# ntc-ai/sliders-conceptmod

Measured on AMD Instinct MI355X. Metric: slider train-steps/sec (4-pass UNet fwd+bwd), higher is better.
Workload: dtype fp16; 1 GPU; sdxl_1024_b2_r4; unet=sdxl, resolution=1024, per_gpu_batch=2, unet_batch=4, global_batch=2, lora_rank=4, train_method=noxattn, network_type=lierla, lora_params=2662400, scheduler=euler_a, parallelism=dp1, pre_roll=excluded, skip_dead_cfg_half=False, dedup_uncond=False, guidance_passes=1 batched UNet call (3 frozen + 1 adapted sub-batches)

## Files before the change

include/smi.h:

```cpp
#ifndef SMI_H_
#define SMI_H_

#include <stddef.h>
#include <stdint.h>

#ifdef __cplusplus
extern "C" {
#endif

#define SMI_MAX_LEVELS 8
#define SMI_DTYPE_F16 0
#define SMI_DTYPE_BF16 1

typedef struct smi_unet_config {
  int dtype;
  int in_channels;
  int out_channels;
  int n_levels;
  int block_out_channels[SMI_MAX_LEVELS];
  int down_has_attn[SMI_MAX_LEVELS];
  int up_has_attn[SMI_MAX_LEVELS];
  int layers_per_block;
  int transformer_layers[SMI_MAX_LEVELS];
  int num_heads[SMI_MAX_LEVELS];
// ... 259 lines not shown
int smi_op_conv3x3(int dtype, const void* in, const void* w_packed, const void* bias, void* out, int nb, int hin,
                   int win, int cin, int cout, int stride, int upsample, int transposed, int hout, int wout,
                   void* stream);
int smi_op_upconv_phase(int dtype, const void* in, const void* w, const void* bias, void* wph, void* planes, void* out, int nb,
                        int h, int w_, int cin, int cout, int tile_code, int* ran_code, void* stream);
int smi_set_upconv_phase(int on);
int smi_op_attention_fwd(int dtype, const void* q, const void* k, const void* v, void* o, float* lse, int b, int h,
                         int nq, int nk, int d, float scale, void* stream);
int smi_op_attention_bwd(int dtype, const void* q, const void* k, const void* v, const void* o, const float* lse,
                         const void* d_o, void* dq, void* dk, void* dv, float* delta, int b, int h, int nq, int nk,
                         int d, float scale, void* stream);
typedef struct smi_attn_args {
  const void *q, *k, *v;
  void* o;
  float* lse;
  const void* d_o;
  void *dq, *dk, *dv;
  float* delta;
  void* stream;
  int64_t ldq, ldk, ldv, ldo, lddo, lddq, lddk, lddv;
  int dtype, b, h, nq, nk, d;
  float scale;
  int causal, sel_xs, sel_fused;
} smi_attn_args;
#define SMI_ATTN_FWD 1
#define SMI_ATTN_XS_FWD 2
#define SMI_ATTN_BWD_FUSED 3
#define SMI_ATTN_DQ 4
#define SMI_ATTN_XS_DQ 5
#define SMI_ATTN_DKV 6
#define SMI_ATTN_DK_DV 7
#define SMI_ATTN_DELTA 8
typedef struct smi_attn_ran {
  int dp;
  int form;
  int n_launches;
  int family[4];
  int chain;
} smi_attn_ran;
int smi_op_attention_ex_fwd(const smi_attn_args* args, smi_attn_ran* ran);
int smi_op_attention_ex_bwd(const smi_attn_args* args, smi_attn_ran* ran);
int smi_op_attention_causal_fwd(int dtype, const void* q, const void* k, const void* v, void* o, float* lse, int b, int h,
                                int n, int d, int64_t ldq, int64_t ldk, int64_t ldv, int64_t ldo, float scale, void* stream);
int smi_op_attention_causal_bwd(int dtype, const void* q, const void* k, const void* v, const void* o, const float* lse,
                                const void* d_o, void* dq, void* dk, void* dv, float* delta, int b, int h, int nq, int nk,
                                int d, int64_t ldq, int64_t ldk, int64_t ldv, int64_t ldo, int64_t lddo, int64_t lddq,
                                int64_t lddk, int64_t lddv, float scale, void* stream);
int smi_op_act(int dtype, const void* x, void* y, const void* dy, void* dx, int64_t n, int kind, void* stream);
int smi_op_groupnorm(int dtype, const void* x, const void* gamma, const void* beta, void* y, const void* dy, void* dx,
                     float* scratch, int nb, int hw, int c, int g, float eps, int silu, void* stream);
int smi_op_layernorm(int dtype, const void* x, const void* gamma, const void* beta, void* y, const void* dy, void* dx,
                     float* mean_rstd, int m, int c, float eps, void* stream);
typedef struct smi_norm_args {
  const void *x, *gamma, *beta;
  void* y;
  const void *dy, *add;
  void* dx;
  float* scratch;
  void* stream;
  int dtype, nb, hw, c, g;
  float eps;
// ... 98 lines not shown
```

sliders_conceptmod_amd/_native.py:

```python
from __future__ import annotations

import ctypes as C
import os
from typing import List, Optional, Sequence

import torch

_HERE = os.path.dirname(os.path.abspath(__file__))
LIB_PATH = os.environ.get("SMI_LIB") or os.path.join(_HERE, "libsmi_hip.so")
SMI_MAX_LEVELS = 8
DTYPE_CODE = {torch.float16: 0, torch.bfloat16: 1}


class SmiError(RuntimeError):
    pass


class UNetConfigC(C.Structure):
    _fields_ = [
        ("dtype", C.c_int), ("in_channels", C.c_int), ("out_channels", C.c_int), ("n_levels", C.c_int),
        ("block_out_channels", C.c_int * SMI_MAX_LEVELS), ("down_has_attn", C.c_int * SMI_MAX_LEVELS),
        ("up_has_attn", C.c_int * SMI_MAX_LEVELS), ("layers_per_block", C.c_int),
        ("transformer_layers", C.c_int * SMI_MAX_LEVELS), ("num_heads", C.c_int * SMI_MAX_LEVELS),
        ("mid_transformer_layers", C.c_int), ("cross_attention_dim", C.c_int), ("norm_num_groups", C.c_int),
# ... 35 lines not shown
    _fields_ = [("name", C.c_char_p), ("data", C.c_void_p), ("ndim", C.c_int), ("shape", C.c_int64 * 4)]


class LoraSiteC(C.Structure):
    _fields_ = [("target", C.c_char_p), ("off_down", C.c_int64), ("off_up", C.c_int64), ("rank", C.c_int),
                ("scale", C.c_float), ("off_dora", C.c_int64)]


class WgradJobC(C.Structure):
    _fields_ = [("X", C.c_void_p), ("P", C.c_void_p), ("dW", C.c_void_p), ("row_scale", C.c_void_p),
                ("ldx", C.c_int64), ("ldp", C.c_int64), ("so_r", C.c_int64), ("so_k", C.c_int64),
                ("M", C.c_int), ("K", C.c_int), ("r", C.c_int), ("seg_cols", C.c_int), ("rows_per_sample", C.c_int),
                ("alpha", C.c_float), ("m_begin", C.c_int), ("conv_tap", C.c_int), ("Hin", C.c_int), ("Win", C.c_int),
                ("Hout", C.c_int), ("Wout", C.c_int), ("conv_stride", C.c_int), ("conv_ups", C.c_int)]


class AttnArgsC(C.Structure):
    _fields_ = [("q", C.c_void_p), ("k", C.c_void_p), ("v", C.c_void_p), ("o", C.c_void_p), ("lse", C.c_void_p),
                ("d_o", C.c_void_p), ("dq", C.c_void_p), ("dk", C.c_void_p), ("dv", C.c_void_p), ("delta", C.c_void_p),
                ("stream", C.c_void_p),
                ("ldq", C.c_int64), ("ldk", C.c_int64), ("ldv", C.c_int64), ("ldo", C.c_int64), ("lddo", C.c_int64),
                ("lddq", C.c_int64), ("lddk", C.c_int64), ("lddv", C.c_int64),
                ("dtype", C.c_int), ("b", C.c_int), ("h", C.c_int), ("nq", C.c_int), ("nk", C.c_int), ("d", C.c_int),
                ("scale", C.c_float), ("causal", C.c_int), ("sel_xs", C.c_int), ("sel_fused", C.c_int)]


class AttnRanC(C.Structure):
    _fields_ = [("dp", C.c_int), ("form", C.c_int), ("n_launches", C.c_int), ("family", C.c_int * 4), ("chain", C.c_int)]


class NormArgsC(C.Structure):
    _fields_ = [("x", C.c_void_p), ("gamma", C.c_void_p), ("beta", C.c_void_p), ("y", C.c_void_p), ("dy", C.c_void_p),
                ("add", C.c_void_p), ("dx", C.c_void_p), ("scratch", C.c_void_p), ("stream", C.c_void_p),
                ("dtype", C.c_int), ("nb", C.c_int), ("hw", C.c_int), ("c", C.c_int), ("g", C.c_int), ("eps", C.c_float),
                ("silu", C.c_int), ("bwd_n0", C.c_int), ("sel_fused", C.c_int)]


class NormRanC(C.Structure):
    _fields_ = [("form", C.c_int), ("chunks", C.c_int), ("slots", C.c_int), ("nv", C.c_int), ("r", C.c_int)]


class DoraSiteC(C.Structure):
    _fields_ = [("W", C.c_void_p), ("off_down", C.c_int64), ("off_up", C.c_int64), ("off_dora", C.c_int64),
                ("dW", C.c_void_p), ("dWt", C.c_void_p), ("cnorm", C.c_void_p), ("r", C.c_int), ("nseg", C.c_int),
                ("K", C.c_int), ("cs", C.c_int), ("scale", C.c_float)]


class LoraPrepSiteC(C.Structure):
    _fields_ = [("off_down", C.c_int64), ("off_up", C.c_int64), ("dst_down", C.c_int64), ("dst_up", C.c_int64),
                ("r", C.c_int), ("nseg", C.c_int), ("K", C.c_int), ("cs", C.c_int), ("rows_pad", C.c_int), ("conv", C.c_int),
                ("dst_gw", C.c_int64)]
# ... 816 lines not shown
```

sliders_conceptmod_amd/build.py:

```python
import os
import subprocess
import sys

HERE = os.path.dirname(os.path.abspath(__file__))
CSRC = os.path.join(HERE, "csrc")
LIB = os.path.join(HERE, "libsmi_hip.so")
SOURCES = ["gemm.hip", "gemm2.hip", "gemm3.hip", "gemm4.hip", "attention.hip", "attention_causal.hip", "norm.hip", "elementwise.hip", "lora.hip", "vae_decode.hip", "clip_vision.hip",
           "lpips.hip", "mmdit.hip", "engine.hip", "engine_unet.hip", "engine_vae.hip", "engine_clip.hip", "engine_lpips.hip", "engine_mmdit.hip", "ops_api.hip"]
FLAGS = ["--offload-arch=gfx950", "-O3", "-std=c++17", "-fPIC"]
EXTRA_FLAGS = {"attention.hip": ["-mllvm", "-amdgpu-mfma-vgpr-form"],
               "attention_causal.hip": ["-mllvm", "-amdgpu-mfma-vgpr-form"]}


def _stale(target, deps):
    if not os.path.exists(target):
        return True
    t = os.path.getmtime(target)
    return any(os.path.getmtime(d) > t for d in deps)


def build(force: bool = False, verbose: bool = False) -> str:
    hipcc = os.environ.get("HIPCC", "hipcc")
    objdir = os.path.join(HERE, "build")
    os.makedirs(objdir, exist_ok=True)
    headers = [os.path.join(CSRC, h) for h in ("smi_common.h", "kernels.h", "gemm_tile.h", "gemm_epilogue.h", "engine.h")] + [
        os.path.join(os.path.dirname(HERE), "include", "smi.h")]
    objs = []
    procs = []
    for src in SOURCES:
        s = os.path.join(CSRC, src)
        o = os.path.join(objdir, src.replace(".hip", ".o"))
        objs.append(o)
        if force or _stale(o, [s] + headers):
            cmd = [hipcc] + FLAGS + EXTRA_FLAGS.get(src, []) + ["-c", s, "-o", o]
            if verbose:
                print(" ".join(cmd))
            procs.append((src, subprocess.Popen(cmd, stdout=subprocess.PIPE, stderr=subprocess.STDOUT)))
    for src, p in procs:
        out, _ = p.communicate()
        if p.returncode != 0:
            raise RuntimeError(f"hipcc failed on {src}:\n{out.decode()}")
    if force or procs or _stale(LIB, objs):
        cmd = [hipcc, "--offload-arch=gfx950", "-shared", "-fPIC", "-o", LIB] + objs
        r = subprocess.run(cmd, stdout=subprocess.PIPE, stderr=subprocess.STDOUT)
        if r.returncode != 0:
            raise RuntimeError(f"link failed:\n{r.stdout.decode()}")
    return LIB

# ... 4 lines not shown
```

sliders_conceptmod_amd/csrc/attention.hip:

```cpp
#include <stdlib.h>

#include <type_traits>

#include "kernels.h"

namespace smi {
namespace {

constexpr float LOG2E = 1.4426950408889634f;
constexpr int TK = 64;
typedef short s16x4 __attribute__((ext_vector_type(4)));
__host__ __device__ constexpr int tr_stride(int DP) { return ((DP * 2) % 128 == 64) ? DP : DP + 32; }

__device__ __forceinline__ void xcd_block(int& bx, int& by, int& bz) {
  const int nx = gridDim.x, ny = gridDim.y;
  const int total = nx * ny * gridDim.z;
  const int lin = blockIdx.x + nx * (blockIdx.y + ny * blockIdx.z);
  const int q = total >> 3, r = total & 7, xcd = lin & 7;
  const int v = (xcd < r ? xcd * (q + 1) : r * (q + 1) + (xcd - r) * q) + (lin >> 3);
  bx = v % nx;
  const int t = v / nx;
  by = t % ny;
  bz = t / ny;
}

template <typename T, int DP>
struct Stage {
  static constexpr int LDN = DP + 8;
  static constexpr int LDV = tr_stride(DP);
  static constexpr int NIT = DP / 32;
  static constexpr int CPR = DP / 8;

  static __device__ __forceinline__ void load(u32x4 (&reg)[NIT], __amdgpu_buffer_rsrc_t r, int64_t row0, int nrows,
                                              int64_t ld, int col0, int D, int tid) {
#pragma unroll
    for (int i = 0; i < NIT; ++i) {
      const int idx = tid + 256 * i;
      const int row = idx / CPR, ch = idx - row * CPR;
      const bool ok = (row0 + row < nrows) && (ch * 8 < D);
      const uint32_t off = ok ? (uint32_t)(((row0 + row) * ld + col0 + ch * 8) * 2) : OOB;
      reg[i] = buf_load16(r, off);
    }
  }
  static __device__ __forceinline__ void store_nat(const u32x4 (&reg)[NIT], T* dst, int tid) {
#pragma unroll
    for (int i = 0; i < NIT; ++i) {
      const int idx = tid + 256 * i;
      const int row = idx / CPR, ch = idx - row * CPR;
      *reinterpret_cast<u32x4*>(dst + row * LDN + ch * 8) = reg[i];
    }
  }
  static __device__ __forceinline__ void store_ld(const u32x4 (&reg)[NIT], T* dst, int ld, int tid) {
#pragma unroll
    for (int i = 0; i < NIT; ++i) {
      const int idx = tid + 256 * i;
      const int row = idx / CPR, ch = idx - row * CPR;
      *reinterpret_cast<u32x4*>(dst + row * ld + ch * 8) = reg[i];
    }
  }
};

template <typename T>
__device__ __forceinline__ typename TT<T>::v8 pack8(const f32x16& a, int s) {
  Pack8<T> t;
#pragma unroll
  for (int j = 0; j < 8; ++j) t.e[j] = from_f<T>(a[8 * s + j]);
  return t.v;
}
template <typename T>
__device__ __forceinline__ typename TT<T>::v8 ld_frag_nat(const T* tile, int ldn, int row, int col) {
  Pack8<T> t;
  t.u = *reinterpret_cast<const u32x4*>(tile + row * ldn + col);
  return t.v;
}
template <typename T>
__device__ __forceinline__ typename TT<T>::v8 ld_frag_trhw(const T* tile, int ld, int idx0, int d0, int lane) {
  const T* a = tile + (idx0 + ((lane & 15) >> 2)) * ld + d0 + ((lane >> 4) & 1) * 16 + 4 * (lane & 3);
  typedef __attribute__((address_space(3))) s16x4 lds_s16x4;
  const s16x4 lo = __builtin_amdgcn_ds_read_tr16_b64_v4i16((lds_s16x4*)a);
  const s16x4 hi = __builtin_amdgcn_ds_read_tr16_b64_v4i16((lds_s16x4*)(a + 8 * ld));
  union {
    s16x4 h[2];
    typename TT<T>::v8 v;
  } u;
  u.h[0] = lo;
  u.h[1] = hi;
  return u.v;
}

template <typename T> struct Sum4;
template <> struct Sum4<f16> {
  static __device__ __forceinline__ f32x4 add8(f16x8 pf, f32x4 acc) {
    const f16x4 one = {(f16)1.f, (f16)1.f, (f16)1.f, (f16)1.f};
    const f16x4 lo = {pf[0], pf[1], pf[2], pf[3]}, hi = {pf[4], pf[5], pf[6], pf[7]};
    acc = __builtin_amdgcn_mfma_f32_4x4x4f16(one, lo, acc, 0, 0, 0);
    return __builtin_amdgcn_mfma_f32_4x4x4f16(one, hi, acc, 0, 0, 0);
  }
};
template <> struct Sum4<bf16> {
  typedef short s4 __attribute__((ext_vector_type(4)));
  static __device__ __forceinline__ f32x4 add8(bf16x8 pf, f32x4 acc) {
    const s4 one = {0x3F80, 0x3F80, 0x3F80, 0x3F80};
    union { bf16x8 v; s4 h[2]; } u;
    u.v = pf;
    acc = __builtin_amdgcn_mfma_f32_4x4x4bf16_1k(one, u.h[0], acc, 0, 0, 0);
    return __builtin_amdgcn_mfma_f32_4x4x4bf16_1k(one, u.h[1], acc, 0, 0, 0);
  }
};
__device__ __forceinline__ void halves_split(float x, float& lo, float& hi) {
  lo = x;
  hi = x;
  asm volatile("s_nop 1\n\tv_permlane32_swap_b32 %0, %1\n\ts_nop 0" : "+v"(lo), "+v"(hi));
}
__device__ __forceinline__ float halves_max(float x) {
  float a, b;
  halves_split(x, a, b);
  return fmaxf(a, b);
}
__device__ __forceinline__ float halves_sum(float x) {
  float a, b;
  halves_split(x, a, b);
  return a + b;
}
__device__ __forceinline__ int acc_row(int r, int h2) { return (r & 3) + 8 * (r >> 2) + 4 * h2; }

template <typename T, int DP, int NSD>
__global__ __launch_bounds__(256) void attn_fwd_kernel(AttnParams p) {
  using S = Stage<T, DP>;
  constexpr int NS = DP / 16, NB = DP / 32;
  constexpr bool EX = NSD > 0;
  __shared__ __attribute__((aligned(16))) T Ks2[2][TK * S::LDN];
  __shared__ __attribute__((aligned(16))) T Vs2[2][TK * S::LDV];

  const int tid = threadIdx.x, lane = tid & 63, wave = tid >> 6;
  const int ql = lane & 31, h2 = lane >> 5;
  int bx, head, b;
  xcd_block(bx, head, b);
  const int q_idx = bx * 128 + wave * 32 + ql;
  const int col0 = head * p.D;
  const int nsd = NSD > 0 ? NSD : (p.D + 15) / 16;

  const auto rQ = make_rsrc((const T*)p.Q + (int64_t)b * p.Nq * p.ldq, (uint32_t)((int64_t)p.Nq * p.ldq * 2));
  const auto rK = make_rsrc((const T*)p.K + (int64_t)b * p.Nk * p.ldk, (uint32_t)((int64_t)p.Nk * p.ldk * 2));
  const auto rV = make_rsrc((const T*)p.V + (int64_t)b * p.Nk * p.ldv, (uint32_t)((int64_t)p.Nk * p.ldv * 2));

  typename TT<T>::v8 qf[NS];
#pragma unroll
// ... 454 lines not shown
#pragma unroll
      for (int g = 0; g < 4; ++g) {
        const int d = i * 32 + 8 * g + 4 * h2;
        if (d < p.D) {
          if (DO_DK) {
            Pack4<T> t;
#pragma unroll
            for (int j = 0; j < 4; ++j) t.e[j] = from_f<T>(dk[i][4 * g + j] * p.scale);
            *reinterpret_cast<u32x2*>((T*)p.dK + ((int64_t)b * p.Nk + k_idx) * p.lddk + col0 + d) = t.u;
          }
          if (DO_DV) {
            Pack4<T> t;
#pragma unroll
            for (int j = 0; j < 4; ++j) t.e[j] = from_f<T>(dv[i][4 * g + j]);
            *reinterpret_cast<u32x2*>((T*)p.dV + ((int64_t)b * p.Nk + k_idx) * p.lddv + col0 + d) = t.u;
          }
        }
      }
  }
}

constexpr int XS_KEYS = 96;

__device__ __forceinline__ void wave_lds_sync() {
  __builtin_amdgcn_fence(__ATOMIC_ACQ_REL, "wavefront");
  __builtin_amdgcn_wave_barrier();
}

template <typename T, int DP>
struct XsTile {
  static constexpr int LDN = DP + 8;
  static constexpr int CPR = DP / 8;
  static constexpr int TOT = 32 * CPR;
  static constexpr int NIT = TOT / 64;
  static_assert(TOT % 64 == 0, "tile depth");
  static __device__ __forceinline__ void rc(int lane, int i, int& row, int& col) {
    const int idx = lane + 64 * i;
    row = idx / CPR;
    col = (idx - row * CPR) * 8;
  }
  static __device__ __forceinline__ void load(u32x4 (&reg)[NIT], __amdgpu_buffer_rsrc_t r, int64_t row0, int nrows,
                                              int64_t ld, int col0, int D, int lane) {
#pragma unroll
    for (int i = 0; i < NIT; ++i) {
      int row, col;
      rc(lane, i, row, col);
      const bool ok = (row0 + row < nrows) && (col < D);
      reg[i] = buf_load16(r, ok ? (uint32_t)(((row0 + row) * ld + col0 + col) * 2) : OOB);
    }
  }
  static __device__ __forceinline__ void to_lds(const u32x4 (&reg)[NIT], T* tile, int lane) {
// ... 346 lines not shown
  constexpr size_t sm = xs_fwd_smem<T, DP>();
  if (sm > 65536) {
    static DynLdsOnce once;
    if (int rc = once.set((const void*)attn_xs_fwd_kernel<T, DP, NSD>, (int)sm)) return rc;
  }
  dim3 grid(xs_grid_x(p), p.H, p.B);
  hipLaunchKernelGGL((attn_xs_fwd_kernel<T, DP, NSD>), grid, dim3(256), sm, st, p);
  SMI_HIP(hipGetLastError());
  return 0;
}
template <typename T, int DP, int NSD>
int xs_dq_launch(const AttnParams& p, hipStream_t st) {
  constexpr size_t sm = xs_dq_smem<T, DP>();
  if (sm > 65536) {
    static DynLdsOnce once;
    if (int rc = once.set((const void*)attn_xs_bwd_dq_kernel<T, DP, NSD>, (int)sm)) return rc;
  }
  dim3 grid(xs_grid_x(p), p.H, p.B);
  hipLaunchKernelGGL((attn_xs_bwd_dq_kernel<T, DP, NSD>), grid, dim3(256), sm, st, p);
  SMI_HIP(hipGetLastError());
  return 0;
}
static int g_sel_xs = -1, g_sel_fused = -1;
static thread_local AttnRan g_ran;
static void ran_begin(int dp, int form) {
  g_ran = AttnRan();
  g_ran.dp = dp;
  g_ran.form = form;
}
static void ran_add(int family, int chain = 0) {
  if (g_ran.n < 4) g_ran.family[g_ran.n] = family;
  ++g_ran.n;
  if (chain) g_ran.chain = chain;
}
static int xs_chain(const AttnParams& p) { return cdiv(p.Nq, 128) / xs_grid_x(p); }

static bool xs_enabled() {
  static const bool on = []() { const char* e = getenv("SMI_ATTN_XS"); return !(e && e[0] == '0'); }();
  return g_sel_xs < 0 ? on : g_sel_xs != 0;
}

template <typename T, int DP>
constexpr size_t dkv_smem() {
  return (size_t)(2 * TK * Stage<T, DP>::LDN + 2 * TK * Stage<T, DP>::LDV) * sizeof(T) + 2 * TK * sizeof(float);
}
template <typename T, int DP, int WHICH, int NSD>
// ... 11 lines not shown
  const int total = gridDim.x, lin = blockIdx.x;
  const int q = total >> 3, r = total & 7, xcd = lin & 7;
  const int v = (xcd < r ? xcd * (q + 1) : r * (q + 1) + (xcd - r) * q) + (lin >> 3);
  const int bh = v / per, j = v - bh * per;
  const int head = bh % p.H, b = bh / p.H;
  if (j < nkb)
    attn_bwd_dkv_body<T, DP, 3, NSD, true>(p, j, head, b, dyn_smem);
  else
    attn_bwd_dq_body<T, DP, NSD, false>(p, j - nkb, head, b, dyn_smem);
}

int check_attn(const AttnParams& p) {
  SMI_CHECK(p.D % 8 == 0 && p.D >= 8 && p.D <= 160, "attention: head_dim %d unsupported (need D %% 8 == 0, <= 160)", p.D);
  SMI_CHECK(p.ldq % 8 == 0 && p.ldk % 8 == 0 && p.ldv % 8 == 0 && p.ldo % 8 == 0,
            "attention: row strides ldq %lld ldk %lld ldv %lld ldo %lld must be multiples of 8 elements (16 bytes)",
            (long long)p.ldq, (long long)p.ldk, (long long)p.ldv, (long long)p.ldo);
  SMI_CHECK(p.B > 0 && p.H > 0 && p.Nq > 0 && p.Nk > 0, "attention: empty shape");
  SMI_CHECK((int64_t)p.Nq * p.ldq * 2 < 0xFFFFFFF0ll && (int64_t)p.Nk * p.ldk * 2 < 0xFFFFFFF0ll, "attention: per-batch tensor larger than 4 GiB");
  return 0;
}

template <int DP> constexpr int alt_steps() { return DP == 64 ? 3 : (DP == 96 ? 5 : 0); }

template <typename T, int DP>
int fwd_t(const AttnParams& p, hipStream_t st) {
  dim3 grid(cdiv(p.Nq, 128), p.H, p.B);
  constexpr int NS = DP / 16, ALT = alt_steps<DP>();
  const int nsd = (p.D + 15) / 16;
  ran_begin(DP, nsd == NS ? 1 : (ALT > 0 && nsd == ALT ? 2 : 0));
  if (p.Nk <= XS_KEYS && xs_enabled() && g_ran.form != 0) {
    ran_add(ATTN_RAN_XS_FWD, xs_chain(p));
    if (nsd == NS) return xs_fwd_launch<T, DP, NS>(p, st);
    return xs_fwd_launch<T, DP, (ALT > 0 ? ALT : NS)>(p, st);
  }
  ran_add(ATTN_RAN_FWD);
  if (nsd == NS)
    hipLaunchKernelGGL((attn_fwd_kernel<T, DP, NS>), grid, dim3(256), 0, st, p);
  else if (ALT > 0 && nsd == ALT)
    hipLaunchKernelGGL((attn_fwd_kernel<T, DP, (ALT > 0 ? ALT : NS)>), grid, dim3(256), 0, st, p);
  else
    hipLaunchKernelGGL((attn_fwd_kernel<T, DP, 0>), grid, dim3(256), 0, st, p);
  SMI_HIP(hipGetLastError());
  return 0;
}

template <typename T, int DP, int WHICH, int NSD>
int dkv_launch(const AttnParams& p, dim3 grid, size_t sm, hipStream_t st) {
  if (sm > 65536) {
    static DynLdsOnce once;
    if (int rc = once.set((const void*)attn_bwd_dkv_kernel<T, DP, WHICH, NSD>, (int)sm)) return rc;
  }
  hipLaunchKernelGGL((attn_bwd_dkv_kernel<T, DP, WHICH, NSD>), grid, dim3(256), sm, st, p);
  return 0;
}

template <typename T, int DP>
int bwd_t(const AttnParams& p, hipStream_t st) {
  constexpr int NS = DP / 16, ALT = alt_steps<DP>();
// ... 57 lines not shown
      else { if (dkv_launch<T, DP, 3, 0>(p, grid, sm, st)) return -2; }
    } else {
      if (form == 1) {
        if (dkv_launch<T, DP, 1, NS>(p, grid, sm, st) || dkv_launch<T, DP, 2, NS>(p, grid, sm, st)) return -2;
      } else {
        if (dkv_launch<T, DP, 1, 0>(p, grid, sm, st) || dkv_launch<T, DP, 2, 0>(p, grid, sm, st)) return -2;
      }
    }
  }
  SMI_HIP(hipGetLastError());
  return 0;
}

template <typename T>
int dispatch(const AttnParams& p, hipStream_t st, bool bwd) {
  if (p.D <= 32) return bwd ? bwd_t<T, 32>(p, st) : fwd_t<T, 32>(p, st);
  if (p.D <= 64) return bwd ? bwd_t<T, 64>(p, st) : fwd_t<T, 64>(p, st);
  if (p.D <= 96) return bwd ? bwd_t<T, 96>(p, st) : fwd_t<T, 96>(p, st);
  return bwd ? bwd_t<T, 160>(p, st) : fwd_t<T, 160>(p, st);
}

}

void set_attn_select(int xs, int fused) {
  g_sel_xs = xs;
  g_sel_fused = fused;
}
AttnRan attn_last_ran() { return g_ran; }

int launch_attn_fwd(const AttnParams& p, hipStream_t stream) {
  g_ran = AttnRan();
  if (check_attn(p)) return -1;
  return p.dtype == DT_F16 ? dispatch<f16>(p, stream, false) : dispatch<bf16>(p, stream, false);
}
int launch_attn_bwd(const AttnParams& p, hipStream_t stream) {
  g_ran = AttnRan();
  if (p.causal) return launch_attn_causal_bwd(p, stream);
  if (check_attn(p)) return -1;
  SMI_CHECK(p.lse && p.delta && p.dO && p.O, "attention bwd: lse/delta/dO/O required");
  SMI_CHECK(p.lddo % 8 == 0 && (!p.dQ || p.lddq % 8 == 0) && (!p.dK || p.lddk % 8 == 0) && (!p.dV || p.lddv % 8 == 0),
            "attention bwd: row strides lddo %lld lddq %lld lddk %lld lddv %lld must be multiples of 8 elements (16 bytes)",
            (long long)p.lddo, (long long)p.lddq, (long long)p.lddk, (long long)p.lddv);
  return p.dtype == DT_F16 ? dispatch<f16>(p, stream, true) : dispatch<bf16>(p, stream, true);
}

}
```

sliders_conceptmod_amd/csrc/kernels.h:

```cpp
#pragma once
#include <vector>

#include "smi_common.h"

namespace smi {

struct GemmParams {
  int dtype = DT_F16;
  const void* A = nullptr;
  int64_t lda = 0;
  const void* W = nullptr;
  void* C = nullptr;
  int64_t ldc = 0;
  int out_f32 = 0;
  int M = 0, N = 0, K = 0;
  const void* bias = nullptr;
  const void* res = nullptr;
  int64_t ldr = 0;
  const void* rowvec = nullptr;
  int rows_per_vec = 1;
  int64_t ld_rowvec = 0;
  const float* lora_xa = nullptr;
  int64_t ld_xa = 0;
  const float* lora_up = nullptr;
// ... 133 lines not shown
void set_gemm_scratch(void* ws, size_t bytes);
bool gemm_geglu_supported(const GemmParams& p);

int launch_conv3x3_small(int dtype, const void* in, const void* w, const void* bias, void* out, int out_f32, int Nb,
                         int H, int W, int Cin, int Cout, hipStream_t stream);

struct AttnParams {
  int dtype = DT_F16;
  const void *Q = nullptr, *K = nullptr, *V = nullptr;
  void* O = nullptr;
  float* lse = nullptr;
  int64_t ldq = 0, ldk = 0, ldv = 0, ldo = 0;
  int B = 0, H = 0, Nq = 0, Nk = 0, D = 0;
  float scale = 1.f;
  int causal = 0;
  const void* dO = nullptr;
  int64_t lddo = 0;
  float* delta = nullptr;
  void *dQ = nullptr, *dK = nullptr, *dV = nullptr;
  int64_t lddq = 0, lddk = 0, lddv = 0;
};
int launch_attn_fwd(const AttnParams& p, hipStream_t stream);
int launch_attn_bwd(const AttnParams& p, hipStream_t stream);
void set_attn_select(int xs, int fused);
enum {
  ATTN_RAN_FWD = 1,
  ATTN_RAN_XS_FWD = 2,
  ATTN_RAN_BWD_FUSED = 3,
  ATTN_RAN_DQ = 4,
  ATTN_RAN_XS_DQ = 5,
  ATTN_RAN_DKV = 6,
  ATTN_RAN_DK_DV = 7,
  ATTN_RAN_DELTA = 8,
};
struct AttnRan {
  int dp = 0;
  int form = 0;
  int n = 0;
  int family[4] = {0, 0, 0, 0};
  int chain = 0;
};
AttnRan attn_last_ran();
int launch_attn_causal_bwd(const AttnParams& p, hipStream_t stream);

int gn_num_chunks(int HW);
size_t gn_partial_floats(int Nb, int HW, int G);
int launch_groupnorm_fwd(int dtype, const void* x, const void* gamma, const void* beta, void* y, float* ab,
                         float* mean_rstd, float* partial, int Nb, int HW, int C, int G, float eps, int silu,
                         hipStream_t stream);
int launch_groupnorm_stats(int dtype, const void* x, const void* gamma, const void* beta, float* ab, float* mean_rstd,
                           float* partial, int Nb, int HW, int C, int G, float eps, hipStream_t stream);
int launch_groupnorm_bwd(int dtype, const void* x, const void* dy, const void* gamma, const void* beta,
                         const float* a, const float* b, const float* mean_rstd, const void* add, void* dx,
                         float* partial, int Nb, int HW, int C, int G, int silu, hipStream_t stream);
void set_gn_select(int fused);
enum {
  NORM_RAN_GN_ONE = 1,
  NORM_RAN_GN_TWO = 2,
  NORM_RAN_GN_FOLD = 3,
  NORM_RAN_LN = 4,
};
struct NormRan {
  int form = 0;
// ... 192 lines not shown
```

sliders_conceptmod_amd/csrc/ops_api.hip:

```cpp
#include <cstdarg>
#include <cstdio>
#include <cstring>
#include <vector>

#include "../../include/smi.h"
#include "kernels.h"

namespace smi {

static thread_local char g_err[2048] = "";
void set_error(const char* fmt, ...) {
  va_list ap;
  va_start(ap, fmt);
  vsnprintf(g_err, sizeof(g_err), fmt, ap);
  va_end(ap);
}

}

using namespace smi;

extern "C" {

const char* smi_last_error(void) { return g_err; }
// ... 151 lines not shown
  p.B = a->b;
  p.H = a->h;
  p.Nq = a->nq;
  p.Nk = a->nk;
  p.D = a->d;
  p.scale = a->scale;
  p.causal = a->causal;
  p.dO = a->d_o;
  p.lddo = a->lddo;
  p.delta = a->delta;
  p.dQ = a->dq;
  p.dK = a->dk;
  p.dV = a->dv;
  p.lddq = a->lddq;
  p.lddk = a->lddk;
  p.lddv = a->lddv;
  return p;
}
static int attn_ex_run(const smi_attn_args* a, smi_attn_ran* ran, bool bwd) {
  if (!a) {
    set_error("smi_op_attention_ex: NULL arguments");
    return -1;
  }
  set_attn_select(a->sel_xs, a->sel_fused);
  const AttnParams p = attn_ex(a);
  const int rc = bwd ? launch_attn_bwd(p, (hipStream_t)a->stream) : launch_attn_fwd(p, (hipStream_t)a->stream);
  set_attn_select(-1, -1);
  if (ran) {
    const AttnRan r = attn_last_ran();
    ran->dp = r.dp;
    ran->form = r.form;
    ran->n_launches = r.n;
    for (int i = 0; i < 4; ++i) ran->family[i] = r.family[i];
    ran->chain = r.chain;
  }
  return rc;
}
int smi_op_attention_ex_fwd(const smi_attn_args* a, smi_attn_ran* ran) { return attn_ex_run(a, ran, false); }
int smi_op_attention_ex_bwd(const smi_attn_args* a, smi_attn_ran* ran) { return attn_ex_run(a, ran, true); }
static AttnParams attn_causal(int dtype, const void* q, const void* k, const void* v, void* o, float* lse, int b, int h, int n,
                              int d, int64_t ldq, int64_t ldk, int64_t ldv, int64_t ldo, float scale) {
  AttnParams p = attn_dense(dtype, q, k, v, o, lse, b, h, n, n, d, scale);
  p.ldq = ldq;
  p.ldk = ldk;
  p.ldv = ldv;
  p.ldo = ldo;
  p.causal = 1;
  return p;
}
int smi_op_attention_causal_fwd(int dtype, const void* q, const void* k, const void* v, void* o, float* lse, int b, int h,
                                int n, int d, int64_t ldq, int64_t ldk, int64_t ldv, int64_t ldo, float scale, void* stream) {
  return launch_attn_fwd(attn_causal(dtype, q, k, v, o, lse, b, h, n, d, ldq, ldk, ldv, ldo, scale), (hipStream_t)stream);
}
int smi_op_attention_causal_bwd(int dtype, const void* q, const void* k, const void* v, const void* o, const float* lse,
                                const void* d_o, void* dq, void* dk, void* dv, float* delta, int b, int h, int nq, int nk,
                                int d, int64_t ldq, int64_t ldk, int64_t ldv, int64_t ldo, int64_t lddo, int64_t lddq,
                                int64_t lddk, int64_t lddv, float scale, void* stream) {
// ... 391 lines not shown
```

Before: 6.756 steps/s.

## Add 8-wave ping-pong attention forward kernel for head_dim 64 fp16

Adds a 512-thread attention forward kernel where two 4-wave groups alternate, one staging the next K/V tiles into double-buffered LDS while the other runs the QK/PV MFMAs. Each block covers 256 queries instead of 128. A rule picks this kernel for fp16, head_dim 64, at least 256 keys and enough workgroups, with an env switch to turn it off. Shared attention helpers move into a common header. The aim is better overlap of global loads with matrix math, at the cost of more register and LDS pressure and added barrier handshakes.

```diff
diff --git a/include/smi.h b/include/smi.h
--- a/include/smi.h
+++ b/include/smi.h
@@ -305,6 +305,7 @@
   int dtype, b, h, nq, nk, d;
   float scale;
   int causal, sel_xs, sel_fused;
+  int sel_fwd;
 } smi_attn_args;
 #define SMI_ATTN_FWD 1
 #define SMI_ATTN_XS_FWD 2
@@ -320,6 +321,7 @@
   int n_launches;
   int family[4];
   int chain;
+  int fwd;
 } smi_attn_ran;
 int smi_op_attention_ex_fwd(const smi_attn_args* args, smi_attn_ran* ran);
 int smi_op_attention_ex_bwd(const smi_attn_args* args, smi_attn_ran* ran);
diff --git a/sliders_conceptmod_amd/_native.py b/sliders_conceptmod_amd/_native.py
--- a/sliders_conceptmod_amd/_native.py
+++ b/sliders_conceptmod_amd/_native.py
@@ -81,11 +81,13 @@
                 ("ldq", C.c_int64), ("ldk", C.c_int64), ("ldv", C.c_int64), ("ldo", C.c_int64), ("lddo", C.c_int64),
                 ("lddq", C.c_int64), ("lddk", C.c_int64), ("lddv", C.c_int64),
                 ("dtype", C.c_int), ("b", C.c_int), ("h", C.c_int), ("nq", C.c_int), ("nk", C.c_int), ("d", C.c_int),
-                ("scale", C.c_float), ("causal", C.c_int), ("sel_xs", C.c_int), ("sel_fused", C.c_int)]
+                ("scale", C.c_float), ("causal", C.c_int), ("sel_xs", C.c_int), ("sel_fused", C.c_int),
+                ("sel_fwd", C.c_int)]
 
 
 class AttnRanC(C.Structure):
-    _fields_ = [("dp", C.c_int), ("form", C.c_int), ("n_launches", C.c_int), ("family", C.c_int * 4), ("chain", C.c_int)]
+    _fields_ = [("dp", C.c_int), ("form", C.c_int), ("n_launches", C.c_int), ("family", C.c_int * 4), ("chain", C.c_int),
+                ("fwd", C.c_int)]
 
 
 class NormArgsC(C.Structure):
diff --git a/sliders_conceptmod_amd/build.py b/sliders_conceptmod_amd/build.py
--- a/sliders_conceptmod_amd/build.py
+++ b/sliders_conceptmod_amd/build.py
@@ -5,10 +5,11 @@
 HERE = os.path.dirname(os.path.abspath(__file__))
 CSRC = os.path.join(HERE, "csrc")
 LIB = os.path.join(HERE, "libsmi_hip.so")
-SOURCES = ["gemm.hip", "gemm2.hip", "gemm3.hip", "gemm4.hip", "attention.hip", "attention_causal.hip", "norm.hip", "elementwise.hip", "lora.hip", "vae_decode.hip", "clip_vision.hip",
+SOURCES = ["gemm.hip", "gemm2.hip", "gemm3.hip", "gemm4.hip", "attention.hip", "attention_fwd8.hip", "attention_causal.hip", "norm.hip", "elementwise.hip", "lora.hip", "vae_decode.hip", "clip_vision.hip",
            "lpips.hip", "mmdit.hip", "engine.hip", "engine_unet.hip", "engine_vae.hip", "engine_clip.hip", "engine_lpips.hip", "engine_mmdit.hip", "ops_api.hip"]
 FLAGS = ["--offload-arch=gfx950", "-O3", "-std=c++17", "-fPIC"]
 EXTRA_FLAGS = {"attention.hip": ["-mllvm", "-amdgpu-mfma-vgpr-form"],
+               "attention_fwd8.hip": ["-mllvm", "-amdgpu-mfma-vgpr-form"],
                "attention_causal.hip": ["-mllvm", "-amdgpu-mfma-vgpr-form"]}
 
 
@@ -23,7 +24,7 @@
     hipcc = os.environ.get("HIPCC", "hipcc")
     objdir = os.path.join(HERE, "build")
     os.makedirs(objdir, exist_ok=True)
-    headers = [os.path.join(CSRC, h) for h in ("smi_common.h", "kernels.h", "gemm_tile.h", "gemm_epilogue.h", "engine.h")] + [
+    headers = [os.path.join(CSRC, h) for h in ("smi_common.h", "kernels.h", "attention_common.h", "gemm_tile.h", "gemm_epilogue.h", "engine.h")] + [
         os.path.join(os.path.dirname(HERE), "include", "smi.h")]
     objs = []
     procs = []
diff --git a/sliders_conceptmod_amd/csrc/attention.hip b/sliders_conceptmod_amd/csrc/attention.hip
--- a/sliders_conceptmod_amd/csrc/attention.hip
+++ b/sliders_conceptmod_amd/csrc/attention.hip
@@ -2,127 +2,10 @@
 
 #include <type_traits>
 
-#include "kernels.h"
+#include "attention_common.h"
 
 namespace smi {
 namespace {
-
-constexpr float LOG2E = 1.4426950408889634f;
-constexpr int TK = 64;
-typedef short s16x4 __attribute__((ext_vector_type(4)));
-__host__ __device__ constexpr int tr_stride(int DP) { return ((DP * 2) % 128 == 64) ? DP : DP + 32; }
-
-__device__ __forceinline__ void xcd_block(int& bx, int& by, int& bz) {
-  const int nx = gridDim.x, ny = gridDim.y;
-  const int total = nx * ny * gridDim.z;
-  const int lin = blockIdx.x + nx * (blockIdx.y + ny * blockIdx.z);
-  const int q = total >> 3, r = total & 7, xcd = lin & 7;
-  const int v = (xcd < r ? xcd * (q + 1) : r * (q + 1) + (xcd - r) * q) + (lin >> 3);
-  bx = v % nx;
-  const int t = v / nx;
-  by = t % ny;
-  bz = t / ny;
-}
-
-template <typename T, int DP>
-struct Stage {
-  static constexpr int LDN = DP + 8;
-  static constexpr int LDV = tr_stride(DP);
-  static constexpr int NIT = DP / 32;
-  static constexpr int CPR = DP / 8;
-
-  static __device__ __forceinline__ void load(u32x4 (&reg)[NIT], __amdgpu_buffer_rsrc_t r, int64_t row0, int nrows,
-                                              int64_t ld, int col0, int D, int tid) {
-#pragma unroll
-    for (int i = 0; i < NIT; ++i) {
-      const int idx = tid + 256 * i;
-      const int row = idx / CPR, ch = idx - row * CPR;
-      const bool ok = (row0 + row < nrows) && (ch * 8 < D);
-      const uint32_t off = ok ? (uint32_t)(((row0 + row) * ld + col0 + ch * 8) * 2) : OOB;
-      reg[i] = buf_load16(r, off);
-    }
-  }
-  static __device__ __forceinline__ void store_nat(const u32x4 (&reg)[NIT], T* dst, int tid) {
-#pragma unroll
-    for (int i = 0; i < NIT; ++i) {
-      const int idx = tid + 256 * i;
-      const int row = idx / CPR, ch = idx - row * CPR;
-      *reinterpret_cast<u32x4*>(dst + row * LDN + ch * 8) = reg[i];
-    }
-  }
-  static __device__ __forceinline__ void store_ld(const u32x4 (&reg)[NIT], T* dst, int ld, int tid) {
-#pragma unroll
-    for (int i = 0; i < NIT; ++i) {
-      const int idx = tid + 256 * i;
-      const int row = idx / CPR, ch = idx - row * CPR;
-      *reinterpret_cast<u32x4*>(dst + row * ld + ch * 8) = reg[i];
-    }
-  }
-};
-
-template <typename T>
-__device__ __forceinline__ typename TT<T>::v8 pack8(const f32x16& a, int s) {
-  Pack8<T> t;
-#pragma unroll
-  for (int j = 0; j < 8; ++j) t.e[j] = from_f<T>(a[8 * s + j]);
-  return t.v;
-}
-template <typename T>
-__device__ __forceinline__ typename TT<T>::v8 ld_frag_nat(const T* tile, int ldn, int row, int col) {
-  Pack8<T> t;
-  t.u = *reinterpret_cast<const u32x4*>(tile + row * ldn + col);
-  return t.v;
-}
-template <typename T>
-__device__ __forceinline__ typename TT<T>::v8 ld_frag_trhw(const T* tile, int ld, int idx0, int d0, int lane) {
-  const T* a = tile + (idx0 + ((lane & 15) >> 2)) * ld + d0 + ((lane >> 4) & 1) * 16 + 4 * (lane & 3);
-  typedef __attribute__((address_space(3))) s16x4 lds_s16x4;
-  const s16x4 lo = __builtin_amdgcn_ds_read_tr16_b64_v4i16((lds_s16x4*)a);
-  const s16x4 hi = __builtin_amdgcn_ds_read_tr16_b64_v4i16((lds_s16x4*)(a + 8 * ld));
-  union {
-    s16x4 h[2];
-    typename TT<T>::v8 v;
-  } u;
-  u.h[0] = lo;
-  u.h[1] = hi;
-  return u.v;
-}
-
-template <typename T> struct Sum4;
-template <> struct Sum4<f16> {
-  static __device__ __forceinline__ f32x4 add8(f16x8 pf, f32x4 acc) {
-    const f16x4 one = {(f16)1.f, (f16)1.f, (f16)1.f, (f16)1.f};
-    const f16x4 lo = {pf[0], pf[1], pf[2], pf[3]}, hi = {pf[4], pf[5], pf[6], pf[7]};
-    acc = __builtin_amdgcn_mfma_f32_4x4x4f16(one, lo, acc, 0, 0, 0);
-    return __builtin_amdgcn_mfma_f32_4x4x4f16(one, hi, acc, 0, 0, 0);
-  }
-};
-template <> struct Sum4<bf16> {
-  typedef short s4 __attribute__((ext_vector_type(4)));
-  static __device__ __forceinline__ f32x4 add8(bf16x8 pf, f32x4 acc) {
-    const s4 one = {0x3F80, 0x3F80, 0x3F80, 0x3F80};
-    union { bf16x8 v; s4 h[2]; } u;
-    u.v = pf;
-    acc = __builtin_amdgcn_mfma_f32_4x4x4bf16_1k(one, u.h[0], acc, 0, 0, 0);
-    return __builtin_amdgcn_mfma_f32_4x4x4bf16_1k(one, u.h[1], acc, 0, 0, 0);
-  }
-};
-__device__ __forceinline__ void halves_split(float x, float& lo, float& hi) {
-  lo = x;
-  hi = x;
-  asm volatile("s_nop 1\n\tv_permlane32_swap_b32 %0, %1\n\ts_nop 0" : "+v"(lo), "+v"(hi));
-}
-__device__ __forceinline__ float halves_max(float x) {
-  float a, b;
-  halves_split(x, a, b);
-  return fmaxf(a, b);
-}
-__device__ __forceinline__ float halves_sum(float x) {
-  float a, b;
-  halves_split(x, a, b);
-  return a + b;
-}
-__device__ __forceinline__ int acc_row(int r, int h2) { return (r & 3) + 8 * (r >> 2) + 4 * h2; }
 
 template <typename T, int DP, int NSD>
 __global__ __launch_bounds__(256) void attn_fwd_kernel(AttnParams p) {
@@ -623,11 +506,6 @@
 
 constexpr int XS_KEYS = 96;
 
-__device__ __forceinline__ void wave_lds_sync() {
-  __builtin_amdgcn_fence(__ATOMIC_ACQ_REL, "wavefront");
-  __builtin_amdgcn_wave_barrier();
-}
-
 template <typename T, int DP>
 struct XsTile {
   static constexpr int LDN = DP + 8;
@@ -1020,6 +898,7 @@
   return 0;
 }
 static int g_sel_xs = -1, g_sel_fused = -1;
+static int g_sel_fwd = 0;
 static thread_local AttnRan g_ran;
 static void ran_begin(int dp, int form) {
   g_ran = AttnRan();
@@ -1077,6 +956,14 @@
 
 template <int DP> constexpr int alt_steps() { return DP == 64 ? 3 : (DP == 96 ? 5 : 0); }
 
+constexpr int FWD8_MIN_KEYS = 256;
+constexpr int FWD8_MIN_WGS = 1024;
+static bool fwd8_rule(const AttnParams& p) {
+  static const bool on = []() { const char* e = getenv("SMI_ATTN_FWD8"); return !(e && e[0] == '0'); }();
+  if (!on || !attn_fwd8_can(p) || p.dtype != DT_F16) return false;
+  return p.Nk >= FWD8_MIN_KEYS && (int64_t)cdiv(p.Nq, 256) * p.H * p.B >= FWD8_MIN_WGS;
+}
+
 template <typename T, int DP>
 int fwd_t(const AttnParams& p, hipStream_t st) {
   dim3 grid(cdiv(p.Nq, 128), p.H, p.B);
@@ -1084,11 +971,21 @@
   const int nsd = (p.D + 15) / 16;
   ran_begin(DP, nsd == NS ? 1 : (ALT > 0 && nsd == ALT ? 2 : 0));
   if (p.Nk <= XS_KEYS && xs_enabled() && g_ran.form != 0) {
+    SMI_CHECK(g_sel_fwd != 2, "attention: the 8-wave forward was pinned, but %d keys go to the single-pass kernel", p.Nk);
     ran_add(ATTN_RAN_XS_FWD, xs_chain(p));
     if (nsd == NS) return xs_fwd_launch<T, DP, NS>(p, st);
     return xs_fwd_launch<T, DP, (ALT > 0 ? ALT : NS)>(p, st);
   }
   ran_add(ATTN_RAN_FWD);
+  if constexpr (DP == 64) {
+    if (g_sel_fwd == 2 || (g_sel_fwd == 0 && fwd8_rule(p))) {
+      g_ran.fwd = 2;
+      const int rc = launch_attn_fwd8(p, st);
+      if (rc) g_ran = AttnRan();
+      return rc;
+    }
+  }
+  g_ran.fwd = 1;
   if (nsd == NS)
     hipLaunchKernelGGL((attn_fwd_kernel<T, DP, NS>), grid, dim3(256), 0, st, p);
   else if (ALT > 0 && nsd == ALT)
@@ -1192,9 +1089,10 @@
 
 }
 
-void set_attn_select(int xs, int fused) {
+void set_attn_select(int xs, int fused, int fwd) {
   g_sel_xs = xs;
   g_sel_fused = fused;
+  g_sel_fwd = fwd;
 }
 AttnRan attn_last_ran() { return g_ran; }
 
diff --git a/sliders_conceptmod_amd/csrc/attention_common.h b/sliders_conceptmod_amd/csrc/attention_common.h
--- /dev/null
+++ b/sliders_conceptmod_amd/csrc/attention_common.h
@@ -0,0 +1,132 @@
+#pragma once
+
+#include "kernels.h"
+
+namespace smi {
+namespace {
+
+constexpr float LOG2E = 1.4426950408889634f;
+constexpr int TK = 64;
+typedef short s16x4 __attribute__((ext_vector_type(4)));
+__host__ __device__ constexpr int tr_stride(int DP) { return ((DP * 2) % 128 == 64) ? DP : DP + 32; }
+
+__device__ __forceinline__ void xcd_block(int& bx, int& by, int& bz) {
+  const int nx = gridDim.x, ny = gridDim.y;
+  const int total = nx * ny * gridDim.z;
+  const int lin = blockIdx.x + nx * (blockIdx.y + ny * blockIdx.z);
+  const int q = total >> 3, r = total & 7, xcd = lin & 7;
+  const int v = (xcd < r ? xcd * (q + 1) : r * (q + 1) + (xcd - r) * q) + (lin >> 3);
+  bx = v % nx;
+  const int t = v / nx;
+  by = t % ny;
+  bz = t / ny;
+}
+
+template <typename T, int DP, int NT = 256>
+struct Stage {
+  static constexpr int LDN = DP + 8;
+  static constexpr int LDV = tr_stride(DP);
+  static constexpr int NIT = TK * DP / 8 / NT;
+  static constexpr int CPR = DP / 8;
+  static_assert(NIT * NT * 8 == TK * DP, "tile chunks must divide among the threads");
+
+  static __device__ __forceinline__ void load(u32x4 (&reg)[NIT], __amdgpu_buffer_rsrc_t r, int64_t row0, int nrows,
+                                              int64_t ld, int col0, int D, int tid) {
+#pragma unroll
+    for (int i = 0; i < NIT; ++i) {
+      const int idx = tid + NT * i;
+      const int row = idx / CPR, ch = idx - row * CPR;
+      const bool ok = (row0 + row < nrows) && (ch * 8 < D);
+      const uint32_t off = ok ? (uint32_t)(((row0 + row) * ld + col0 + ch * 8) * 2) : OOB;
+      reg[i] = buf_load16(r, off);
+    }
+  }
+  static __device__ __forceinline__ void store_nat(const u32x4 (&reg)[NIT], T* dst, int tid) {
+#pragma unroll
+    for (int i = 0; i < NIT; ++i) {
+      const int idx = tid + NT * i;
+      const int row = idx / CPR, ch = idx - row * CPR;
+      *reinterpret_cast<u32x4*>(dst + row * LDN + ch * 8) = reg[i];
+    }
+  }
+  static __device__ __forceinline__ void store_ld(const u32x4 (&reg)[NIT], T* dst, int ld, int tid) {
+#pragma unroll
+    for (int i = 0; i < NIT; ++i) {
+      const int idx = tid + NT * i;
+      const int row = idx / CPR, ch = idx - row * CPR;
+      *reinterpret_cast<u32x4*>(dst + row * ld + ch * 8) = reg[i];
+    }
+  }
+};
+
+template <typename T>
+__device__ __forceinline__ typename TT<T>::v8 pack8(const f32x16& a, int s) {
+  Pack8<T> t;
+#pragma unroll
+  for (int j = 0; j < 8; ++j) t.e[j] = from_f<T>(a[8 * s + j]);
+  return t.v;
+}
+template <typename T>
+__device__ __forceinline__ typename TT<T>::v8 ld_frag_nat(const T* tile, int ldn, int row, int col) {
+  Pack8<T> t;
+  t.u = *reinterpret_cast<const u32x4*>(tile + row * ldn + col);
+  return t.v;
+}
+template <typename T>
+__device__ __forceinline__ typename TT<T>::v8 ld_frag_trhw(const T* tile, int ld, int idx0, int d0, int lane) {
+  const T* a = tile + (idx0 + ((lane & 15) >> 2)) * ld + d0 + ((lane >> 4) & 1) * 16 + 4 * (lane & 3);
+  typedef __attribute__((address_space(3))) s16x4 lds_s16x4;
+  const s16x4 lo = __builtin_amdgcn_ds_read_tr16_b64_v4i16((lds_s16x4*)a);
+  const s16x4 hi = __builtin_amdgcn_ds_read_tr16_b64_v4i16((lds_s16x4*)(a + 8 * ld));
+  union {
+    s16x4 h[2];
+    typename TT<T>::v8 v;
+  } u;
+  u.h[0] = lo;
+  u.h[1] = hi;
+  return u.v;
+}
+
+template <typename T> struct Sum4;
+template <> struct Sum4<f16> {
+  static __device__ __forceinline__ f32x4 add8(f16x8 pf, f32x4 acc) {
+    const f16x4 one = {(f16)1.f, (f16)1.f, (f16)1.f, (f16)1.f};
+    const f16x4 lo = {pf[0], pf[1], pf[2], pf[3]}, hi = {pf[4], pf[5], pf[6], pf[7]};
+    acc = __builtin_amdgcn_mfma_f32_4x4x4f16(one, lo, acc, 0, 0, 0);
+    return __builtin_amdgcn_mfma_f32_4x4x4f16(one, hi, acc, 0, 0, 0);
+  }
+};
+template <> struct Sum4<bf16> {
+  typedef short s4 __attribute__((ext_vector_type(4)));
+  static __device__ __forceinline__ f32x4 add8(bf16x8 pf, f32x4 acc) {
+    const s4 one = {0x3F80, 0x3F80, 0x3F80, 0x3F80};
+    union { bf16x8 v; s4 h[2]; } u;
+    u.v = pf;
+    acc = __builtin_amdgcn_mfma_f32_4x4x4bf16_1k(one, u.h[0], acc, 0, 0, 0);
+    return __builtin_amdgcn_mfma_f32_4x4x4bf16_1k(one, u.h[1], acc, 0, 0, 0);
+  }
+};
+__device__ __forceinline__ void halves_split(float x, float& lo, float& hi) {
+  lo = x;
+  hi = x;
+  asm volatile("s_nop 1\n\tv_permlane32_swap_b32 %0, %1\n\ts_nop 0" : "+v"(lo), "+v"(hi));
+}
+__device__ __forceinline__ float halves_max(float x) {
+  float a, b;
+  halves_split(x, a, b);
+  return fmaxf(a, b);
+}
+__device__ __forceinline__ float halves_sum(float x) {
+  float a, b;
+  halves_split(x, a, b);
+  return a + b;
+}
+__device__ __forceinline__ int acc_row(int r, int h2) { return (r & 3) + 8 * (r >> 2) + 4 * h2; }
+
+__device__ __forceinline__ void wave_lds_sync() {
+  __builtin_amdgcn_fence(__ATOMIC_ACQ_REL, "wavefront");
+  __builtin_amdgcn_wave_barrier();
+}
+
+}
+}
diff --git a/sliders_conceptmod_amd/csrc/attention_fwd8.hip b/sliders_conceptmod_amd/csrc/attention_fwd8.hip
--- /dev/null
+++ b/sliders_conceptmod_amd/csrc/attention_fwd8.hip
@@ -0,0 +1,257 @@
+#include <type_traits>
+
+#include "attention_common.h"
+
+namespace smi {
+namespace {
+
+template <typename T, bool TWO>
+__global__ __launch_bounds__(512, TWO ? 4 : 2) void attn_fwd8_kernel(AttnParams p) {
+  constexpr int DP = 64, NS = DP / 16, NB = DP / 32;
+  using S = Stage<T, DP, 512>;
+  static_assert(S::NIT == 1 && S::CPR == 8, "tile chunks and threads");
+  __shared__ __attribute__((aligned(16))) T Ks2[2][TK * S::LDN];
+  __shared__ __attribute__((aligned(16))) T Vs2[2][TK * S::LDV];
+  constexpr int LDO = DP + 8;
+  static_assert(4 * 32 * LDO <= 2 * TK * S::LDN && 4 * 32 * LDO <= 2 * TK * S::LDV, "the O tiles of a group fit the K / V slots");
+
+  const int tid = threadIdx.x, lane = tid & 63;
+  const int wave = __builtin_amdgcn_readfirstlane(tid >> 6);
+  const int grp = wave >> 2, gi = wave & 3;
+  const int ql = lane & 31, h2 = lane >> 5;
+  int bx, head, b;
+  xcd_block(bx, head, b);
+  const int q0 = bx * 256 + wave * 32;
+  const int q_idx = q0 + ql;
+  const int col0 = head * DP;
+
+  const auto rQ = make_rsrc((const T*)p.Q + (int64_t)b * p.Nq * p.ldq, (uint32_t)((int64_t)p.Nq * p.ldq * 2));
+  const auto rK = make_rsrc((const T*)p.K + (int64_t)b * p.Nk * p.ldk, (uint32_t)((int64_t)p.Nk * p.ldk * 2));
+  const auto rV = make_rsrc((const T*)p.V + (int64_t)b * p.Nk * p.ldv, (uint32_t)((int64_t)p.Nk * p.ldv * 2));
+  const int ntiles = (p.Nk + TK - 1) / TK;
+
+  const int srow = tid >> 3;
+  const uint32_t vk0 = (uint32_t)((srow * p.ldk + col0 + (tid & 7) * 8) * 2), kstep = (uint32_t)(TK * p.ldk * 2);
+  const uint32_t vv0 = (uint32_t)((srow * p.ldv + col0 + (tid & 7) * 8) * 2), vstep = (uint32_t)(TK * p.ldv * 2);
+  T* const ks_w = &Ks2[0][0] + srow * S::LDN + (tid & 7) * 8;
+  T* const vs_w = &Vs2[0][0] + srow * S::LDV + (tid & 7) * 8;
+  auto load_k = [&](int tile) { return buf_load16(rK, tile * TK + srow < p.Nk ? vk0 + (uint32_t)tile * kstep : OOB); };
+  auto load_v = [&](int tile) { return buf_load16(rV, tile * TK + srow < p.Nk ? vv0 + (uint32_t)tile * vstep : OOB); };
+  auto put_k = [&](int tile, u32x4 v) { *reinterpret_cast<u32x4*>(ks_w + (tile & 1) * (TK * S::LDN)) = v; };
+  auto put_v = [&](int tile, u32x4 v) { *reinterpret_cast<u32x4*>(vs_w + (tile & 1) * (TK * S::LDV)) = v; };
+
+  typename TT<T>::v8 qf[NS];
+#pragma unroll
+  for (int s = 0; s < NS; ++s) {
+    Pack8<T> t;
+    t.u = buf_load16(rQ, q_idx < p.Nq ? (uint32_t)(((int64_t)q_idx * p.ldq + col0 + 16 * s + 8 * h2) * 2) : OOB);
+    qf[s] = t.v;
+  }
+  u32x4 rk = load_k(0), rv = load_v(0);
+  {
+    u32x4 rk1 = rk;
+    if (ntiles > 1) rk1 = load_k(1);
+    put_k(0, rk);
+    put_v(0, rv);
+    if (ntiles > 1) put_k(1, rk1);
+  }
+  if (ntiles > 2) rk = load_k(2);
+  if (ntiles > 1) rv = load_v(1);
+  const float sl = p.scale * LOG2E;
+
+  f32x16 o[NB];
+#pragma unroll
+  for (int i = 0; i < NB; ++i)
+#pragma unroll
+    for (int r = 0; r < 16; ++r) o[i][r] = 0.f;
+  float m_run = -INFINITY;
+  f32x4 l4 = {0.f, 0.f, 0.f, 0.f};
+  constexpr bool LSE_F32 = std::is_same<T, bf16>::value;
+  float lx = 0.f;
+  f32x16 st[2];
+  typename TT<T>::v8 pf[4];
+
+  typename TT<T>::v8 kfr[2][NS], vfr[4][NB];
+  auto ld_k = [&](int kt) {
+    const T* Ks = Ks2[kt & 1];
+#pragma unroll
+    for (int sub = 0; sub < 2; ++sub)
+#pragma unroll
+      for (int s = 0; s < NS; ++s) kfr[sub][s] = ld_frag_nat<T>(Ks, S::LDN, sub * 32 + ql, 16 * s + 8 * h2);
+  };
+  auto ld_v = [&](int kt) {
+    const T* Vs = Vs2[kt & 1];
+#pragma unroll
+    for (int sub = 0; sub < 2; ++sub)
+#pragma unroll
+      for (int s2 = 0; s2 < 2; ++s2)
+#pragma unroll
+        for (int i = 0; i < NB; ++i)
+          vfr[sub * 2 + s2][i] = ld_frag_trhw<T>(Vs, S::LDV, sub * 32 + s2 * 16 + 4 * h2, i * 32, lane);
+  };
+  auto mm_s = [&]() {
+#pragma unroll
+    for (int sub = 0; sub < 2; ++sub) {
+#pragma unroll
+      for (int r = 0; r < 16; ++r) st[sub][r] = 0.f;
+#pragma unroll
+      for (int s = 0; s < NS; ++s) st[sub] = TT<T>::mfma32(kfr[sub][s], qf[s], st[sub]);
+    }
+  };
+  auto mm_pv = [&]() {
+#pragma unroll
+    for (int j = 0; j < 4; ++j)
+#pragma unroll
+      for (int i = 0; i < NB; ++i) o[i] = TT<T>::mfma32(vfr[j][i], pf[j], o[i]);
+  };
+  auto mm_rs = [&](int kt) {
+    const T* Ks = Ks2[kt & 1];
+#pragma unroll
+    for (int sub = 0; sub < 2; ++sub) {
+#pragma unroll
+      for (int r = 0; r < 16; ++r) st[sub][r] = 0.f;
+#pragma unroll
+      for (int s = 0; s < NS; ++s)
+        st[sub] = TT<T>::mfma32(ld_frag_nat<T>(Ks, S::LDN, sub * 32 + ql, 16 * s + 8 * h2), qf[s], st[sub]);
+    }
+  };
+  auto mm_rpv = [&](int kt) {
+    const T* Vs = Vs2[kt & 1];
+#pragma unroll
+    for (int j = 0; j < 4; ++j)
+#pragma unroll
+      for (int i = 0; i < NB; ++i)
+        o[i] = TT<T>::mfma32(ld_frag_trhw<T>(Vs, S::LDV, j * 16 + 4 * h2, i * 32, lane), pf[j], o[i]);
+  };
+  auto seg_x = [&](int kt) {
+    const int k0 = kt * TK;
+    if (k0 + TK > p.Nk) {
+      const int lim = p.Nk - k0 - 4 * h2;
+#pragma unroll
+      for (int sub = 0; sub < 2; ++sub)
+#pragma unroll
+        for (int r = 0; r < 16; ++r) {
+          if (sub * 32 + acc_row(r, 0) >= lim) st[sub][r] = -INFINITY;
+          if ((r & 3) == 3) __builtin_amdgcn_sched_barrier(0);
+        }
+    }
+    float ml[2] = {-INFINITY, -INFINITY};
+#pragma unroll
+    for (int sub = 0; sub < 2; ++sub)
+#pragma unroll
+      for (int r = 0; r < 16; ++r) ml[sub] = fmaxf(ml[sub], st[sub][r]);
+    const float mloc = halves_max(fmaxf(ml[0], ml[1]));
+    const bool need = (mloc - m_run) * sl > 8.f;
+    if (__builtin_amdgcn_ballot_w64(need)) {
+      const float m_new = need ? mloc : m_run;
+      const float alpha = __builtin_amdgcn_exp2f((m_run - m_new) * sl);
+      m_run = m_new;
+      l4 *= alpha;
+      if constexpr (LSE_F32) lx *= alpha;
+#pragma unroll
+      for (int i = 0; i < NB; ++i)
+#pragma unroll
+        for (int r = 0; r < 16; ++r) o[i][r] *= alpha;
+    }
+    const float mb = m_run * sl;
+#pragma unroll
+    for (int sub = 0; sub < 2; ++sub) {
+#pragma unroll
+      for (int r = 0; r < 16; ++r) st[sub][r] = __builtin_amdgcn_exp2f(st[sub][r] * sl - mb);
+      if constexpr (LSE_F32) {
+#pragma unroll
+        for (int r = 0; r < 16; ++r) lx += st[sub][r];
+      }
+#pragma unroll
+      for (int s2 = 0; s2 < 2; ++s2) {
+        pf[sub * 2 + s2] = pack8<T>(st[sub], s2);
+        l4 = Sum4<T>::add8(pf[sub * 2 + s2], l4);
+      }
+    }
+  };
+  auto store_o = [&](T* tile) {
+    const float l_tot = halves_sum(l4[0]);
+    const float inv = 1.f / l_tot;
+    float l_lse = l_tot;
+    if constexpr (LSE_F32) l_lse = halves_sum(lx);
+#pragma unroll
+    for (int i = 0; i < NB; ++i)
+#pragma unroll
+      for (int g = 0; g < 4; ++g) {
+        Pack4<T> t;
+#pragma unroll
+        for (int j = 0; j < 4; ++j) t.e[j] = from_f<T>(o[i][4 * g + j] * inv);
+        *reinterpret_cast<u32x2*>(tile + ql * LDO + i * 32 + 8 * g + 4 * h2) = t.u;
+      }
+    wave_lds_sync();
+    const auto rO = make_rsrc((T*)p.O + (int64_t)b * p.Nq * p.ldo, (uint32_t)((int64_t)p.Nq * p.ldo * 2));
+#pragma unroll
+    for (int it = 0; it < 32 * (DP / 8) / 64; ++it) {
+      const int idx = lane + 64 * it;
+      const int row = idx / (DP / 8), col = (idx - row * (DP / 8)) * 8;
+      const u32x4 v = *reinterpret_cast<const u32x4*>(tile + row * LDO + col);
+      buf_store16(rO, q0 + row < p.Nq ? (uint32_t)(((int64_t)(q0 + row) * p.ldo + col0 + col) * 2) : OOB, v);
+    }
+    if (p.lse && h2 == 0 && q_idx < p.Nq)
+      p.lse[((int64_t)b * p.H + head) * p.Nq + q_idx] = m_run * p.scale + __logf(l_lse);
+  };
+
+  auto stage = [&](int t) {
+    if (t + 2 < ntiles) put_k(t + 2, rk);
+    if (t + 1 < ntiles) put_v(t + 1, rv);
+    if (t + 3 < ntiles) rk = load_k(t + 3);
+    if (t + 2 < ntiles) rv = load_v(t + 2);
+  };
+
+  __syncthreads();
+  if (grp == 1) __syncthreads();
+  if constexpr (TWO) {
+    mm_rs(0);
+  } else {
+    ld_k(0);
+    mm_s();
+  }
+  __syncthreads();
+  for (int t = 0; t < ntiles; ++t) {
+    if (grp == 1) stage(t);
+    if constexpr (!TWO) {
+      ld_v(t);
+      if (t + 1 < ntiles) ld_k(t + 1);
+      __builtin_amdgcn_sched_barrier(0);
+    }
+    seg_x(t);
+    __syncthreads();
+    if (grp == 0) stage(t);
+    if constexpr (TWO) {
+      mm_rpv(t);
+      if (t + 1 < ntiles) mm_rs(t + 1);
+    } else {
+      mm_pv();
+      if (t + 1 < ntiles) mm_s();
+    }
+    __syncthreads();
+  }
+  store_o(&Ks2[0][0] + gi * 32 * LDO);
+  if (grp == 0) __syncthreads();
+}
+
+}
+
+bool attn_fwd8_can(const AttnParams& p) {
+  return p.D == 64 && !p.causal && (p.dtype == DT_F16 || p.dtype == DT_BF16) &&
+         (int64_t)p.Nq * p.ldo * 2 < 0xFFFFFFF0ll && (int64_t)p.Nk * p.ldv * 2 < 0xFFFFFFF0ll;
+}
+
+int launch_attn_fwd8(const AttnParams& p, hipStream_t st) {
+  SMI_CHECK(attn_fwd8_can(p), "attention: the 8-wave forward takes head_dim 64 without a mask (head_dim %d, causal %d)", p.D,
+            p.causal);
+  dim3 grid(cdiv(p.Nq, 256), p.H, p.B);
+  if (p.dtype == DT_F16)
+    hipLaunchKernelGGL((attn_fwd8_kernel<f16, true>), grid, dim3(512), 0, st, p);
+  else
+    hipLaunchKernelGGL((attn_fwd8_kernel<bf16, false>), grid, dim3(512), 0, st, p);
+  SMI_HIP(hipGetLastError());
+  return 0;
+}
+
+}
diff --git a/sliders_conceptmod_amd/csrc/kernels.h b/sliders_conceptmod_amd/csrc/kernels.h
--- a/sliders_conceptmod_amd/csrc/kernels.h
+++ b/sliders_conceptmod_amd/csrc/kernels.h
@@ -179,7 +179,9 @@
 };
 int launch_attn_fwd(const AttnParams& p, hipStream_t stream);
 int launch_attn_bwd(const AttnParams& p, hipStream_t stream);
-void set_attn_select(int xs, int fused);
+void set_attn_select(int xs, int fused, int fwd = 0);
+bool attn_fwd8_can(const AttnParams& p);
+int launch_attn_fwd8(const AttnParams& p, hipStream_t stream);
 enum {
   ATTN_RAN_FWD = 1,
   ATTN_RAN_XS_FWD = 2,
@@ -196,6 +198,7 @@
   int n = 0;
   int family[4] = {0, 0, 0, 0};
   int chain = 0;
+  int fwd = 0;
 };
 AttnRan attn_last_ran();
 int launch_attn_causal_bwd(const AttnParams& p, hipStream_t stream);
diff --git a/sliders_conceptmod_amd/csrc/ops_api.hip b/sliders_conceptmod_amd/csrc/ops_api.hip
--- a/sliders_conceptmod_amd/csrc/ops_api.hip
+++ b/sliders_conceptmod_amd/csrc/ops_api.hip
@@ -197,7 +197,11 @@
     set_error("smi_op_attention_ex: NULL arguments");
     return -1;
   }
-  set_attn_select(a->sel_xs, a->sel_fused);
+  if (a->sel_fwd < 0 || a->sel_fwd > 2) {
+    set_error("smi_op_attention_ex: sel_fwd must be 0 (the rule), 1 (4-wave) or 2 (8-wave)");
+    return -1;
+  }
+  set_attn_select(a->sel_xs, a->sel_fused, a->sel_fwd);
   const AttnParams p = attn_ex(a);
   const int rc = bwd ? launch_attn_bwd(p, (hipStream_t)a->stream) : launch_attn_fwd(p, (hipStream_t)a->stream);
   set_attn_select(-1, -1);
@@ -208,6 +212,7 @@
     ran->n_launches = r.n;
     for (int i = 0; i < 4; ++i) ran->family[i] = r.family[i];
     ran->chain = r.chain;
+    ran->fwd = r.fwd;
   }
   return rc;
 }
```

Result: no change. 6.775 steps/s (median of 6 runs) (+0.3%).
